# madsjulia/GeostatInversion.jl

Measured on AMD Instinct MI355X. Metric: randSVD GB/s + top-k singular-value rel-err, n=1e6 rank=256, higher is better.
Workload: dtype f64

## Files before the change

### geostatinversion.jl_amd/csrc/panel_lu_blocks.hip

```cpp
#include "panel_lu_dev.hpp"
#include <type_traits>

namespace gsi { namespace hipk {

template <int K>
__device__ inline void u12_stage_L11(double* L11, const double* __restrict__ Y, int64_t ld, int64_t jb, int64_t jbrow) {
#pragma unroll 8
  for (int e = threadIdx.x; e < K * K; e += 256) {
    const int r = e % K, c = e / K;
    L11[r * K + c] = Y[(jbrow + r) + (jb + c) * ld];
  }
}
template <int K>
__device__ inline void u12_solve(const double* L11, double (&x)[K]) {
#pragma unroll
  for (int r = 1; r < K; ++r) {
    double v = x[r];
#pragma unroll
    for (int p = 0; p < r; ++p) v -= L11[r * K + p] * x[p];
    x[r] = v;
  }
}

template <int K>
__global__ __launch_bounds__(256) void lu_u12_kernel(const double* __restrict__ Y, int64_t ld, int64_t jb, int64_t jbrow,
                                                     int64_t c0, int64_t c1, double* __restrict__ out) {
  __shared__ double L11[K * K];
  u12_stage_L11<K>(L11, Y, ld, jb, jbrow);
  __syncthreads();
  if (threadIdx.x >= 64) return;
  const int64_t c = c0 + (int64_t)blockIdx.x * 64 + threadIdx.x;
  if (c >= c1) return;
  double x[K];
  const double* col = Y + jbrow + c * ld;
#pragma unroll
  for (int r = 0; r < K; ++r) x[r] = col[r];
  u12_solve<K>(L11, x);
  double* o = out + (c - c0) * K;
#pragma unroll
  for (int r = 0; r < K; ++r) o[r] = x[r];
}

template <int K, int DEPTH, int RK_CHUNK>
__global__ __launch_bounds__(256) __attribute__((amdgpu_waves_per_eu(RK_CHUNK == 64 ? 3 : 2, RK_CHUNK == 64 ? 3 : 4))) void lu_rankk_kernel(double* __restrict__ Y, int64_t ld, int64_t m, int64_t r_begin,
                                                       int64_t jb, int64_t c0, int64_t t,
                                                       const double* __restrict__ U12) {
  typedef double double4_t __attribute__((ext_vector_type(4)));
  constexpr int KP = K + 2;
  extern __shared__ double us[];
  const int tid = threadIdx.x, lane = tid & 63, wave = tid >> 6;
  const int jl = lane & 15, kk = lane >> 4;
  const int64_t rb = r_begin + ((int64_t)blockIdx.x * 4 + wave) * 32;
  double fa[2][K / 4];
#pragma unroll
  for (int h = 0; h < 2; ++h) {
    const int64_t rrow = rb + 16 * h + jl;
#pragma unroll
    for (int s = 0; s < K / 4; ++s) fa[h][s] = (rrow < m) ? Y[rrow + (jb + 4 * s + kk) * ld] : 0.0;
  }
  for (int64_t cc0 = 0; cc0 < t; cc0 += RK_CHUNK) {
    const int tc = (int)((t - cc0 < RK_CHUNK) ? (t - cc0) : RK_CHUNK);
    __syncthreads();
    for (int e = tid; e < RK_CHUNK * K; e += 256) {
      const int k = e % K, c = e / K;
      us[c * KP + k] = (c < tc) ? U12[k + (cc0 + c) * K] : 0.0;
    }
    __syncthreads();
    if (rb >= m) continue;
    const int ntile = (tc + 15) / 16;
    double cin[2][4];
    auto load_tile = [&](int tt, double (&dst)[2][4]) {
#pragma unroll
      for (int h = 0; h < 2; ++h) {
        const int64_t rrow = rb + 16 * h + jl;
#pragma unroll
        for (int reg = 0; reg < 4; ++reg) {
          const int cl = 16 * tt + kk + 4 * reg;
          dst[h][reg] = (rrow < m && cl < tc) ? Y[rrow + (c0 + cc0 + cl) * ld] : 0.0;
        }
      }
    };
    load_tile(0, cin);
    double cin2[2][4];
    if (DEPTH == 2 && ntile > 1) load_tile(1, cin2);
    for (int tt = 0; tt < ntile; ++tt) {
      double4_t acc[2];
#pragma unroll
      for (int h = 0; h < 2; ++h) acc[h] = (double4_t){cin[h][0], cin[h][1], cin[h][2], cin[h][3]};
      if (DEPTH == 2) {
#pragma unroll
        for (int h = 0; h < 2; ++h)
#pragma unroll
          for (int reg = 0; reg < 4; ++reg) cin[h][reg] = cin2[h][reg];
        if (tt + 2 < ntile) load_tile(tt + 2, cin2);
      } else if (tt + 1 < ntile) load_tile(tt + 1, cin);
#pragma unroll
      for (int s = 0; s < K / 4; ++s) {
        const double fb = -us[(16 * tt + jl) * KP + 4 * s + kk];
#pragma unroll
        for (int h = 0; h < 2; ++h) acc[h] = __builtin_amdgcn_mfma_f64_16x16x4f64(fb, fa[h][s], acc[h], 0, 0, 0);
      }
#pragma unroll
      for (int h = 0; h < 2; ++h) {
        const int64_t rrow = rb + 16 * h + jl;
#pragma unroll
        for (int reg = 0; reg < 4; ++reg) {
          const int cl = 16 * tt + kk + 4 * reg;
          if (rrow < m && cl < tc) Y[rrow + (c0 + cc0 + cl) * ld] = acc[h][reg];
        }
      }
    }
  }
}

template <int K, int DEPTH, int CHUNK>
static void launch_rankk_v(hipStream_t st, unsigned grid, double* Y, int64_t ld, int64_t m, int64_t r_begin, int64_t jb,
                           int64_t c0, int64_t t, const double* U12) {
  constexpr size_t shmem = (size_t)CHUNK * (K + 2) * sizeof(double);
  static std::atomic<uint64_t> attr_mask{0};
  if (first_use_on_this_device(attr_mask))
    (void)hipFuncSetAttribute((const void*)lu_rankk_kernel<K, DEPTH, CHUNK>, hipFuncAttributeMaxDynamicSharedMemorySize, (int)shmem);
  hipLaunchKernelGGL((lu_rankk_kernel<K, DEPTH, CHUNK>), dim3(grid), dim3(256), shmem, st, Y, ld, m, r_begin, jb, c0, t, U12);
}
template <int K>
static void launch_rankk(hipStream_t st, unsigned grid, double* Y, int64_t ld, int64_t m, int64_t r_begin, int64_t jb,
                         int64_t c0, int64_t t, const double* U12) {
  static const int depth = getenv("GSI_LU_RK_DEPTH") ? atoi(getenv("GSI_LU_RK_DEPTH")) : 1;
  static const int chunk = getenv("GSI_LU_RK_CHUNK") ? atoi(getenv("GSI_LU_RK_CHUNK")) : 64;
  if (chunk == 64 && depth == 2) launch_rankk_v<K, 2, 64>(st, grid, Y, ld, m, r_begin, jb, c0, t, U12);
  else if (chunk == 64) launch_rankk_v<K, 1, 64>(st, grid, Y, ld, m, r_begin, jb, c0, t, U12);
  else if (depth == 2) launch_rankk_v<K, 2, 128>(st, grid, Y, ld, m, r_begin, jb, c0, t, U12);
  else launch_rankk_v<K, 1, 128>(st, grid, Y, ld, m, r_begin, jb, c0, t, U12);
}

constexpr int LL_WAVES = 12;
constexpr int LL_BS = 64 * LL_WAVES;
constexpr size_t LL_LDS = (size_t)4 * 64 * 66 * sizeof(double);
template <int NB>
constexpr int ll_group() { return (int)(LL_LDS / ((size_t)NB * (NB + 2) * sizeof(double))); }

__device__ __forceinline__ char* ll_advance(char* p, int64_t step) {
  p += step;
  asm volatile("" : "+s"(p));
  return p;
}

template <int NB, bool WIDE>
__global__ __launch_bounds__(LL_BS) void lu_leftlook_kernel(double* __restrict__ Y, int64_t ld, int64_t m, int64_t jb, int tc,
                                                            int ip0, int ip1, const double* __restrict__ U12, int64_t ldu) {
  typedef double double4_t __attribute__((ext_vector_type(4)));
  typedef typename std::conditional<WIDE, uint64_t, uint32_t>::type off_t;
  constexpr int KP = NB + 2, NT = NB / 16, NS = NB / 4;
  extern __shared__ double us[];
  const int tid = threadIdx.x, lane = tid & 63;
  const int wave = __builtin_amdgcn_readfirstlane(tid >> 6);
  const int jl = lane & 15, kk = lane >> 4;
  const int nbk = ip1 - ip0;
  for (int e = tid; e < nbk * NB * NB; e += LL_BS) {
    const int k = e % NB, c = (e / NB) % NB, q = e / (NB * NB);
    us[(q * NB + c) * KP + k] = (c < tc) ? -U12[(int64_t)(ip0 + q) * ldu + (jb + c) * NB + k] : 0.0;
  }
  __syncthreads();
  const int lb = jl * KP + kk;
  const int64_t nch = (m - jb + 15) / 16;
  const int64_t cs = ld * (int64_t)sizeof(double);
  for (int64_t ch = (int64_t)blockIdx.x * LL_WAVES + wave; ch < nch; ch += (int64_t)gridDim.x * LL_WAVES) {
    const int64_t rb = jb + ch * 16;
    const int64_t r = (rb + jl < m) ? rb + jl : m - 1;
    const off_t vo = (off_t)((r - rb) * (int64_t)sizeof(double) + kk * cs);
    auto at = [&](char* colp) -> double* { return reinterpret_cast<double*>(colp + vo); };
    char* const cbase = reinterpret_cast<char*>(Y + rb + jb * ld);
    double4_t acc[NT];
    {
      char* p = cbase;
#pragma unroll
      for (int tt = 0; tt < NT; ++tt)
#pragma unroll
        for (int reg = 0; reg < 4; ++reg) {
          acc[tt][reg] = (16 * tt + 4 * reg + kk < tc) ? *at(p) : 0.0;
          p = ll_advance(p, 4 * cs);
        }
    }
    double fa[NS], fn[NS];
    char* pf = reinterpret_cast<char*>(Y + rb + (int64_t)ip0 * NB * ld);
    auto load_frag = [&](double (&f)[NS]) {
#pragma unroll
      for (int s = 0; s < NS; ++s) {
        f[s] = *at(pf);
        pf = ll_advance(pf, 4 * cs);
      }
    };
    auto run = [&](const double (&f)[NS], int q) {
      const double* ub = us + (q - ip0) * NB * KP + lb;
#pragma unroll
      for (int s = 0; s < NS; ++s)
#pragma unroll
        for (int tt = 0; tt < NT; ++tt)
          acc[tt] = __builtin_amdgcn_mfma_f64_16x16x4f64(ub[16 * tt * KP + 4 * s], f[s], acc[tt], 0, 0, 0);
    };
    load_frag(fa);
    int q = ip0;
    for (; q + 1 < ip1; ++q) {
      load_frag(fn);
      run(fa, q);
#pragma unroll
      for (int s = 0; s < NS; ++s) fa[s] = fn[s];
    }
    run(fa, q);
    const bool live = rb + jl < m;
    char* p = cbase;
#pragma unroll
    for (int tt = 0; tt < NT; ++tt)
#pragma unroll
      for (int reg = 0; reg < 4; ++reg) {
        if (live && 16 * tt + 4 * reg + kk < tc) *at(p) = acc[tt][reg];
        p = ll_advance(p, 4 * cs);
      }
  }
}

template <int K>
__global__ __launch_bounds__(256) void lu_urows_kernel(const double* __restrict__ Y, int64_t ld, int64_t jb, int nprev,
                                                       int64_t c0, int64_t c1, const double* __restrict__ U12, int64_t ldu,
                                                       double* __restrict__ out) {
  typedef double double4_t __attribute__((ext_vector_type(4)));
  constexpr int TP = K + 1;
  __shared__ double L11[K * K];
  __shared__ double T[64 * TP];
  u12_stage_L11<K>(L11, Y, ld, jb, jb);
  const int tid = threadIdx.x, lane = tid & 63, wave = tid >> 6;
  const int jl = lane & 15, kk = lane >> 4;
  const int64_t cb = c0 + (int64_t)blockIdx.x * 64;
  if (wave < K / 16) {
    const int64_t row = jb + 16 * wave + jl;
    double4_t acc[4];
#pragma unroll
    for (int tt = 0; tt < 4; ++tt)
#pragma unroll
      for (int reg = 0; reg < 4; ++reg) {
        const int64_t c = cb + 16 * tt + kk + 4 * reg;
        acc[tt][reg] = (c < c1) ? Y[row + c * ld] : 0.0;
      }
    for (int q = 0; q < nprev; ++q) {
      const double* ub = U12 + (int64_t)q * ldu;
#pragma unroll
      for (int s = 0; s < K / 4; ++s) {
        const double fa = Y[row + ((int64_t)q * K + 4 * s + kk) * ld];
#pragma unroll
        for (int tt = 0; tt < 4; ++tt) {
          const int64_t c = cb + 16 * tt + jl;
          const double fb = (c < c1) ? -ub[c * K + 4 * s + kk] : 0.0;
          acc[tt] = __builtin_amdgcn_mfma_f64_16x16x4f64(fb, fa, acc[tt], 0, 0, 0);
        }
      }
    }
#pragma unroll
    for (int tt = 0; tt < 4; ++tt)
#pragma unroll
      for (int reg = 0; reg < 4; ++reg) T[(16 * tt + kk + 4 * reg) * TP + 16 * wave + jl] = acc[tt][reg];
  }
  __syncthreads();
  if (tid >= 64) return;
  const int64_t c = cb + tid;
  if (c >= c1) return;
  double x[K];
#pragma unroll
  for (int r = 0; r < K; ++r) x[r] = T[tid * TP + r];
  u12_solve<K>(L11, x);
  double* o = out + (c - c0) * K;
#pragma unroll
  for (int r = 0; r < K; ++r) o[r] = x[r];
}

template <int NB, bool WIDE>
static void launch_leftlook_v(hipStream_t st, unsigned grid, double* Y, int64_t ld, int64_t m, int64_t jb, int tc,
                              const double* U12, int64_t ldu) {
  static std::atomic<uint64_t> attr_mask{0};
  if (first_use_on_this_device(attr_mask))
    (void)hipFuncSetAttribute((const void*)lu_leftlook_kernel<NB, WIDE>, hipFuncAttributeMaxDynamicSharedMemorySize, (int)LL_LDS);
  const int nprev = (int)(jb / NB);
  for (int ip0 = 0; ip0 < nprev; ip0 += ll_group<NB>()) {
    const int ip1 = std::min(nprev, ip0 + ll_group<NB>());
    const size_t shmem = (size_t)(ip1 - ip0) * NB * (NB + 2) * sizeof(double);
    hipLaunchKernelGGL((lu_leftlook_kernel<NB, WIDE>), dim3(grid), dim3(LL_BS), shmem, st, Y, ld, m, jb, tc, ip0, ip1, U12, ldu);
  }
}
static void lu_ll_update(hipStream_t st, double* Y, int64_t ld, int64_t m, int64_t l, int64_t jb, int b, int nb,
                         const double* u12) {
  if (jb == 0 || m <= jb) return;
  int dev = 0, ncu = 0;
  (void)hipGetDevice(&dev);
  if (hipDeviceGetAttribute(&ncu, hipDeviceAttributeMultiprocessorCount, dev) != hipSuccess || ncu < 1) ncu = 256;
  const int64_t chunks = (m - jb + 15) / 16;
  const unsigned grid = (unsigned)std::min<int64_t>((chunks + LL_WAVES - 1) / LL_WAVES, ncu);
  const bool wide = (3 * ld + 32) * (int64_t)sizeof(double) >= ((int64_t)1 << 32);
  const int64_t ldu = (int64_t)nb * l;
  if (nb == 64) {
    if (wide) launch_leftlook_v<64, true>(st, grid, Y, ld, m, jb, b, u12, ldu);
    else launch_leftlook_v<64, false>(st, grid, Y, ld, m, jb, b, u12, ldu);
  } else {
    if (wide) launch_leftlook_v<32, true>(st, grid, Y, ld, m, jb, b, u12, ldu);
    else launch_leftlook_v<32, false>(st, grid, Y, ld, m, jb, b, u12, ldu);
  }
}
static void lu_ll_urows(hipStream_t st, const double* Y, int64_t ld, int64_t l, int64_t jb, int nb, double* u12) {
  const int64_t c0 = jb + nb, ldu = (int64_t)nb * l;
  if (c0 >= l) return;
  const unsigned gu = (unsigned)((l - c0 + 63) / 64);
  double* out = u12 + (jb / nb) * ldu + c0 * nb;
  if (nb == 64) {
    if (jb == 0) hipLaunchKernelGGL(lu_u12_kernel<64>, dim3(gu), dim3(256), 0, st, Y, ld, jb, jb, c0, l, out);
    else hipLaunchKernelGGL(lu_urows_kernel<64>, dim3(gu), dim3(256), 0, st, Y, ld, jb, (int)(jb / nb), c0, l, u12, ldu, out);
  } else {
    if (jb == 0) hipLaunchKernelGGL(lu_u12_kernel<32>, dim3(gu), dim3(256), 0, st, Y, ld, jb, jb, c0, l, out);
    else hipLaunchKernelGGL(lu_urows_kernel<32>, dim3(gu), dim3(256), 0, st, Y, ld, jb, (int)(jb / nb), c0, l, u12, ldu, out);
  }
}

__global__ void lu2_extract_L_kernel(double* __restrict__ Y, int64_t ld, int64_t l) {
  const int64_t total = l * l;
  for (int64_t e = (int64_t)blockIdx.x * blockDim.x + threadIdx.x; e < total; e += (int64_t)gridDim.x * blockDim.x) {
    const int64_t r = e % l, c = e / l;
    if (r == c) Y[r + c * ld] = 1.0;
    else if (r < c) Y[r + c * ld] = 0.0;
  }
}

void lu_blocks(hipStream_t st, double* Y, int64_t ld, int64_t m, int64_t l, int nb, double* u12, const LuLeafFn& leaf) {
  for (int64_t jb = 0; jb < l; jb += nb) {
    const int b = (int)((l - jb < nb) ? (l - jb) : nb);
    lu_ll_update(st, Y, ld, m, l, jb, b, nb, u12);
    for (int64_t j0 = jb; j0 < jb + b; j0 += LW) leaf(jb, b, j0, (int)((jb + b - j0 < LW) ? (jb + b - j0) : LW));
    lu_ll_urows(st, Y, ld, l, jb, nb, u12);
  }
  int eb = (int)((l * l + 255) / 256);
  if (eb > 1024) eb = 1024;
  hipLaunchKernelGGL(lu2_extract_L_kernel, dim3(eb), dim3(256), 0, st, Y, ld, l);
}

void lus_u12_block(hipStream_t st, const double* Y, int64_t ld, int64_t row0, int64_t jb, int b, int64_t c0, int64_t c1,
                   double* U12) {
  const unsigned gu = (unsigned)((c1 - c0 + 63) / 64);
  if (b == 64) hipLaunchKernelGGL(lu_u12_kernel<64>, dim3(gu), dim3(256), 0, st, Y, ld, jb, jb - row0, c0, c1, U12);
  else hipLaunchKernelGGL(lu_u12_kernel<32>, dim3(gu), dim3(256), 0, st, Y, ld, jb, jb - row0, c0, c1, U12);
}
void lus_rankk(hipStream_t st, double* Y, int64_t ld, int64_t mloc, int64_t row0, int64_t jb, int b, int64_t c0, int64_t t,
               const double* U12) {
  int64_t rbeg = c0 - row0;
  if (rbeg < 0) rbeg = 0;
  const int64_t mr = mloc - rbeg;
  if (mr <= 0) return;
  const unsigned gr = (unsigned)((mr + 127) / 128);
  if (b == 64) launch_rankk<64>(st, gr, Y, ld, mloc, rbeg, jb, c0, t, U12);
  else launch_rankk<32>(st, gr, Y, ld, mloc, rbeg, jb, c0, t, U12);
}

}}
```

Baseline: 1681.

## Software-pipeline left-look and U-rows LU kernels with prefetch and LDS staging

The left-looking update kernel now prefetches the next chunk's C tile and first L fragment before running the current chunk's last MFMA step. sched_barrier calls keep these loads ahead of the compute, so global latency overlaps MFMA work across chunk iterations. The U-rows kernel now stages each U12 panel through double-buffered LDS with coalesced register prefetch of the next panel and L fragment, replacing strided global loads inside the MFMA loop. The cost is more VGPR pressure, extra shared memory and a __syncthreads per panel, which may reduce occupancy.

Result: no change. 1685 (median of 6 runs) (+0.2%).

```diff
diff --git a/geostatinversion.jl_amd/csrc/panel_lu_blocks.hip b/geostatinversion.jl_amd/csrc/panel_lu_blocks.hip
--- a/geostatinversion.jl_amd/csrc/panel_lu_blocks.hip
+++ b/geostatinversion.jl_amd/csrc/panel_lu_blocks.hip
@@ -144,6 +144,7 @@
   asm volatile("" : "+s"(p));
   return p;
 }
+typedef __attribute__((address_space(1))) double ll_global_double;
 
 template <int NB, bool WIDE>
 __global__ __launch_bounds__(LL_BS) void lu_leftlook_kernel(double* __restrict__ Y, int64_t ld, int64_t m, int64_t jb, int tc,
@@ -164,32 +165,42 @@
   const int lb = jl * KP + kk;
   const int64_t nch = (m - jb + 15) / 16;
   const int64_t cs = ld * (int64_t)sizeof(double);
-  for (int64_t ch = (int64_t)blockIdx.x * LL_WAVES + wave; ch < nch; ch += (int64_t)gridDim.x * LL_WAVES) {
-    const int64_t rb = jb + ch * 16;
+  const int64_t step = (int64_t)gridDim.x * LL_WAVES;
+  int64_t ch = (int64_t)blockIdx.x * LL_WAVES + wave;
+  if (ch >= nch) return;
+  auto lane_off = [&](int64_t rb) -> off_t {
     const int64_t r = (rb + jl < m) ? rb + jl : m - 1;
-    const off_t vo = (off_t)((r - rb) * (int64_t)sizeof(double) + kk * cs);
-    auto at = [&](char* colp) -> double* { return reinterpret_cast<double*>(colp + vo); };
-    char* const cbase = reinterpret_cast<char*>(Y + rb + jb * ld);
+    return (off_t)((r - rb) * (int64_t)sizeof(double) + kk * cs);
+  };
+  auto at = [](char* colp, off_t vo) -> ll_global_double* { return (ll_global_double*)(colp + vo); };
+  auto load_c = [&](double (&c)[4 * NT], int64_t rb, off_t vo) {
+    char* p = reinterpret_cast<char*>(Y + rb + jb * ld);
+#pragma unroll
+    for (int i = 0; i < 4 * NT; ++i) {
+      c[i] = (4 * i + kk < tc) ? *at(p, vo) : 0.0;
+      p = ll_advance(p, 4 * cs);
+    }
+  };
+  char* pf;
+  auto load_frag = [&](double (&f)[NS], off_t vo) {
+#pragma unroll
+    for (int s = 0; s < NS; ++s) {
+      f[s] = *at(pf, vo);
+      pf = ll_advance(pf, 4 * cs);
+    }
+  };
+  int64_t rb = jb + ch * 16;
+  off_t vo = lane_off(rb);
+  double cn[4 * NT], fa[NS], fn[NS];
+  load_c(cn, rb, vo);
+  pf = reinterpret_cast<char*>(Y + rb + (int64_t)ip0 * NB * ld);
+  load_frag(fa, vo);
+#pragma unroll
+  for (int s = 0; s < NS; ++s) asm volatile("" : "+v"(fa[s]));
+  for (;;) {
     double4_t acc[NT];
-    {
-      char* p = cbase;
-#pragma unroll
-      for (int tt = 0; tt < NT; ++tt)
-#pragma unroll
-        for (int reg = 0; reg < 4; ++reg) {
-          acc[tt][reg] = (16 * tt + 4 * reg + kk < tc) ? *at(p) : 0.0;
-          p = ll_advance(p, 4 * cs);
-        }
-    }
-    double fa[NS], fn[NS];
-    char* pf = reinterpret_cast<char*>(Y + rb + (int64_t)ip0 * NB * ld);
-    auto load_frag = [&](double (&f)[NS]) {
-#pragma unroll
-      for (int s = 0; s < NS; ++s) {
-        f[s] = *at(pf);
-        pf = ll_advance(pf, 4 * cs);
-      }
-    };
+#pragma unroll
+    for (int tt = 0; tt < NT; ++tt) acc[tt] = (double4_t){cn[4 * tt], cn[4 * tt + 1], cn[4 * tt + 2], cn[4 * tt + 3]};
     auto run = [&](const double (&f)[NS], int q) {
       const double* ub = us + (q - ip0) * NB * KP + lb;
 #pragma unroll
@@ -198,24 +209,41 @@
         for (int tt = 0; tt < NT; ++tt)
           acc[tt] = __builtin_amdgcn_mfma_f64_16x16x4f64(ub[16 * tt * KP + 4 * s], f[s], acc[tt], 0, 0, 0);
     };
-    load_frag(fa);
     int q = ip0;
     for (; q + 1 < ip1; ++q) {
-      load_frag(fn);
+      load_frag(fn, vo);
       run(fa, q);
 #pragma unroll
       for (int s = 0; s < NS; ++s) fa[s] = fn[s];
     }
-    run(fa, q);
+    const int64_t chn = ch + step, rbn = jb + chn * 16;
+    const bool more = chn < nch;
+    const off_t von = lane_off(rbn);
+    if (more) {
+      load_c(cn, rbn, von);
+      pf = reinterpret_cast<char*>(Y + rbn + (int64_t)ip0 * NB * ld);
+      load_frag(fn, von);
+      __builtin_amdgcn_sched_barrier(0);
+      run(fa, q);
+      __builtin_amdgcn_sched_barrier(0);
+#pragma unroll
+      for (int s = 0; s < NS; ++s) fa[s] = fn[s];
+    } else {
+      run(fa, q);
+    }
     const bool live = rb + jl < m;
-    char* p = cbase;
+    char* p = reinterpret_cast<char*>(Y + rb + jb * ld);
 #pragma unroll
     for (int tt = 0; tt < NT; ++tt)
 #pragma unroll
       for (int reg = 0; reg < 4; ++reg) {
-        if (live && 16 * tt + 4 * reg + kk < tc) *at(p) = acc[tt][reg];
+        if (live && 16 * tt + 4 * reg + kk < tc) *at(p, vo) = acc[tt][reg];
         p = ll_advance(p, 4 * cs);
       }
+    if (!more) break;
+    ch = chn;
+    rb = rbn;
+    vo = von;
   }
 }
 
@@ -225,35 +253,75 @@
                                                        double* __restrict__ out) {
   typedef double double4_t __attribute__((ext_vector_type(4)));
   constexpr int TP = K + 1;
+  constexpr int KP = K + 2, NS = K / 4, NU = 64 * K / 256;
   __shared__ double L11[K * K];
   __shared__ double T[64 * TP];
-  u12_stage_L11<K>(L11, Y, ld, jb, jb);
+  __shared__ double us[2][64 * KP];
   const int tid = threadIdx.x, lane = tid & 63, wave = tid >> 6;
   const int jl = lane & 15, kk = lane >> 4;
   const int64_t cb = c0 + (int64_t)blockIdx.x * 64;
-  if (wave < K / 16) {
-    const int64_t row = jb + 16 * wave + jl;
-    double4_t acc[4];
+  const bool mm = wave < K / 16;
+  const int64_t row = jb + 16 * (mm ? wave : 0) + jl;
+  double4_t acc[4];
+  double ur[NU], fa[NS], fn[NS];
+  const int ulim = (int)((c1 - cb < 64) ? (c1 - cb) : 64) * K;
+  auto load_u = [&](int q) {
+    const double* ub = U12 + (int64_t)q * ldu + cb * K;
+#pragma unroll
+    for (int i = 0; i < NU; ++i) {
+      const int e = tid + 256 * i;
+      ur[i] = ub[e < ulim ? e : 0];
+    }
+  };
+  auto load_l = [&](double (&f)[NS], int q) {
+#pragma unroll
+    for (int s = 0; s < NS; ++s) f[s] = Y[row + ((int64_t)q * K + 4 * s + kk) * ld];
+  };
+  double cr[16];
+  if (mm) {
+#pragma unroll
+    for (int i = 0; i < 16; ++i) {
+      const int64_t c = cb + 4 * i + kk;
+      cr[i] = Y[row + (c < c1 ? c : c1 - 1) * ld];
+    }
+  }
+  load_u(0);
+  if (mm) load_l(fa, 0);
+  __builtin_amdgcn_sched_barrier(0);
+  u12_stage_L11<K>(L11, Y, ld, jb, jb);
+  if (mm) {
 #pragma unroll
     for (int tt = 0; tt < 4; ++tt)
 #pragma unroll
-      for (int reg = 0; reg < 4; ++reg) {
-        const int64_t c = cb + 16 * tt + kk + 4 * reg;
-        acc[tt][reg] = (c < c1) ? Y[row + c * ld] : 0.0;
+      for (int reg = 0; reg < 4; ++reg) acc[tt][reg] = (cb + 16 * tt + 4 * reg + kk < c1) ? cr[4 * tt + reg] : 0.0;
+  }
+  for (int q = 0; q < nprev; ++q) {
+    double* ui = us[q & 1];
+#pragma unroll
+    for (int i = 0; i < NU; ++i) {
+      const int e = tid + 256 * i;
+      ui[(e / K) * KP + e % K] = (e < ulim) ? -ur[i] : 0.0;
+    }
+    __syncthreads();
+    if (q + 1 < nprev) {
+      load_u(q + 1);
+      if (mm) load_l(fn, q + 1);
+    }
+    __builtin_amdgcn_sched_barrier(0);
+    if (mm) {
+      const double* ub = ui + jl * KP + kk;
+#pragma unroll
+      for (int s = 0; s < NS; ++s)
+#pragma unroll
+        for (int tt = 0; tt < 4; ++tt)
+          acc[tt] = __builtin_amdgcn_mfma_f64_16x16x4f64(ub[16 * tt * KP + 4 * s], fa[s], acc[tt], 0, 0, 0);
+      if (q + 1 < nprev) {
+#pragma unroll
+        for (int s = 0; s < NS; ++s) fa[s] = fn[s];
       }
-    for (int q = 0; q < nprev; ++q) {
-      const double* ub = U12 + (int64_t)q * ldu;
-#pragma unroll
-      for (int s = 0; s < K / 4; ++s) {
-        const double fa = Y[row + ((int64_t)q * K + 4 * s + kk) * ld];
-#pragma unroll
-        for (int tt = 0; tt < 4; ++tt) {
-          const int64_t c = cb + 16 * tt + jl;
-          const double fb = (c < c1) ? -ub[c * K + 4 * s + kk] : 0.0;
-          acc[tt] = __builtin_amdgcn_mfma_f64_16x16x4f64(fb, fa, acc[tt], 0, 0, 0);
-        }
-      }
-    }
+    }
+  }
+  if (mm) {
 #pragma unroll
     for (int tt = 0; tt < 4; ++tt)
 #pragma unroll
```
